# microsoft/VidTok

Hardware: AMD Instinct MI355X
Metric: encode+decode frames/sec, vidtok_kl_causal_488_4chn 17x256x256 (higher is better)
Workload: dtype bf16; 1 GPU; vidtok_kl_causal_488_4chn forward (encode+KL+decode), bf16, B=4 clips/GPU, 17x256x256; global_batch=4, launch=hipGraph replay (engine graph cache)

## Files before the change

### vidtok_amd/build.py

```python
import hashlib
import os
import re
import shutil
import subprocess
import sys

HERE = os.path.dirname(os.path.abspath(__file__))
CSRC = os.path.join(HERE, "csrc")
LIB = os.path.join(HERE, "libvidtok_amd.so")
SOURCES = ["conv_igemm_bf16.hip", "conv_igemm_f16.hip", "conv_igemm_f32.hip", "conv_igemm_x3.hip", "conv_igemm_act.hip", "conv_igemm.hip", "conv_in8.hip", "conv_ws2.hip", "conv_narrow.hip", "tblock_ws128.hip", "attention.hip", "pointwise.hip", "groupnorm.hip", "regularizers.hip", "metrics.hip", "lpips.hip", "lpips_grad.hip", "video_io.hip", "segments.hip", "grad.hip", "grad_decoder.hip", "patchgan.hip", "packing.hip", "error.cpp", "options.cpp", "model.cpp"]
HEADERS = ["common.h", "conv_common.h", "conv_rows.h", "conv_select.h", "conv_igemm_kernel.h", "launch.h", "options.h", "row8.h", os.path.join("..", "..", "include", "vidtok_amd.h")]
FLAGS = ["--offload-arch=gfx950", "-O3", "-std=c++17", "-fPIC", "-Wall", "-Wno-unused-function"]
EXTRA_FLAGS = {"conv_ws2.hip": ["-fno-slp-vectorize"], "tblock_ws128.hip": ["-fno-slp-vectorize"]}


NO_SPILL = {"tblock_ws128.hip": "tblock_pair_kernel", "conv_ws2.hip": "conv3x3_ws2_kernel", "conv_in8.hip": "conv_in8_kernel",
            "conv_igemm_bf16.hip": re.compile(r"conv_igemm_glds_kernel.*Lb[01]ELi2ELb0ELi\dELi0EEEvNS_8ConvArgsE$"),
            "conv_igemm_f16.hip": re.compile(r"conv_igemm_glds_kernel.*Lb[01]ELi2ELb0ELi\dELi0EEEvNS_8ConvArgsE$")}
PROF_LAST = ("tblock_pair_kernel", "conv3x3_ws2_kernel")
LLVM_BIN = "/opt/rocm/lib/llvm/bin"


def kernel_resources(obj):
    import re
    import tempfile
    with tempfile.TemporaryDirectory() as d:
        fat, dev = os.path.join(d, "fat.bin"), os.path.join(d, "dev.o")
        subprocess.check_call([f"{LLVM_BIN}/llvm-objcopy", "--dump-section", f".hip_fatbin={fat}", obj])
        subprocess.check_call([f"{LLVM_BIN}/clang-offload-bundler", "--unbundle", "--type=o", f"--input={fat}",
                               "--targets=hipv4-amdgcn-amd-amdhsa--gfx950", f"--output={dev}"])
        notes = subprocess.check_output([f"{LLVM_BIN}/llvm-readelf", "--notes", dev], text=True)
    out = []
    for blk in notes.split("- .agpr_count:")[1:]:
        g = lambda k: re.search(r"\." + k + r":\s+(\S+)", blk).group(1)
        out.append((g("name"), int(g("vgpr_count")), int(blk.split()[0]), int(g("vgpr_spill_count")), int(g("private_segment_fixed_size"))))
    return out


def check_no_spill(objdir):
    if not all(os.path.exists(os.path.join(LLVM_BIN, t)) for t in ("llvm-objcopy", "clang-offload-bundler", "llvm-readelf")):
        print("[vidtok_amd.build] spill check skipped: LLVM binutils not found under", LLVM_BIN, flush=True)
        return
    bad = []
    for src, kern in NO_SPILL.items():
        obj = os.path.join(objdir, os.path.splitext(src)[0] + ".o")
        for name, _v, _a, spill, scratch in kernel_resources(obj):
            measured = any(k in name for k in PROF_LAST) and name.endswith(("Lb1EEEvNS_10TBlockArgsE", "Lb1EEEvNS_8ConvArgsE"))
            hit = kern in name if isinstance(kern, str) else kern.search(name) is not None
            if hit and not measured and (spill or scratch):
                bad.append(f"{name}: {spill} spilled registers, {scratch} B scratch")
    if bad:
        raise RuntimeError("register spills in hand-scheduled kernels (wrong results, not only slow):\n  " + "\n  ".join(bad))


def _hipcc():
    for c in (os.environ.get("HIPCC"), shutil.which("hipcc"), "/opt/rocm/bin/hipcc"):
        if c and os.path.exists(c):
            return c
    raise RuntimeError("hipcc not found (set HIPCC)")


def _src_digest(src):
    h = hashlib.sha256()
    for f in [src] + HEADERS:
        with open(os.path.join(CSRC, f), "rb") as fh:
            h.update(fh.read())
    h.update(" ".join(FLAGS + EXTRA_FLAGS.get(src, [])).encode())
    return h.hexdigest()


def _digest():
    h = hashlib.sha256()
    for src in SOURCES:
        h.update(_src_digest(src).encode())
    return h.hexdigest()


def build(force: bool = False, verbose: bool = True) -> str:
    stamp = LIB + ".stamp"
    dig = _digest()
    if not force and os.path.exists(LIB) and os.path.exists(stamp) and open(stamp).read() == dig:
        return LIB
    hipcc = _hipcc()
    objdir = os.path.join(HERE, "build")
    os.makedirs(objdir, exist_ok=True)
    objs = []
    procs = []
    for src in SOURCES:
        obj = os.path.join(objdir, os.path.splitext(src)[0] + ".o")
        objs.append(obj)
        ostamp, odig = obj + ".stamp", _src_digest(src)
        if not force and os.path.exists(obj) and os.path.exists(ostamp) and open(ostamp).read() == odig:
            continue
        if os.path.exists(ostamp):
            os.remove(ostamp)
        cmd = [hipcc, *FLAGS, *EXTRA_FLAGS.get(src, []), "-x", "hip", "-c", os.path.join(CSRC, src), "-o", obj]
        if verbose:
            print("[vidtok_amd.build]", " ".join(cmd), flush=True)
        procs.append((src, subprocess.Popen(cmd), ostamp, odig))
    failed = []
    for src, p, ostamp, odig in procs:
        if p.wait() != 0:
            failed.append(src)
        else:
            with open(ostamp, "w") as f:
                f.write(odig)
    if failed:
        raise RuntimeError(f"hipcc failed on {', '.join(failed)}")
    check_no_spill(objdir)
    cmd = [hipcc, "--offload-arch=gfx950", "-shared", "-fPIC", *objs, "-o", LIB]
    if verbose:
        print("[vidtok_amd.build]", " ".join(cmd), flush=True)
    subprocess.check_call(cmd)
    with open(stamp, "w") as f:
        f.write(dig)
    return LIB


if __name__ == "__main__":
    build(force="--force" in sys.argv)
    print(LIB)
```

### vidtok_amd/csrc/attention.hip

```cpp
#include <atomic>

#include "conv_common.h"

namespace {

constexpr int FA_D = 512;
constexpr int FA_BQ = 64;
constexpr int FA_BK = 32;
constexpr int FA_KTILE = FA_BK * FA_D * 2;
constexpr int FA_VTILE = FA_D * FA_BK * 2;
constexpr int FA_STAGE = FA_KTILE + FA_VTILE;
constexpr int FA_LDS = 2 * FA_STAGE;

struct FlashArgs {
  const uint16_t* q;
  const uint16_t* k;
  const uint16_t* vt;
  const float* bias_v;
  uint16_t* o;
  int S, ldv;
  float scale_log2e;
};

template <typename H>
__global__ __launch_bounds__(256, 1) void flash_attn_kernel(const FlashArgs p) {
#if defined(__HIP_DEVICE_COMPILE__)
  extern __shared__ __attribute__((aligned(16))) char smem[];
  typedef __attribute__((address_space(3))) void* lds_ptr_t;
  const int lane = threadIdx.x & 63;
  const int wave = __builtin_amdgcn_readfirstlane(threadIdx.x >> 6);
  const int z = blockIdx.y, q0 = blockIdx.x * FA_BQ + wave * 16;
  const int S = p.S;
  const int n = lane & 15, g = lane >> 4;
  const uint16_t* qz = p.q + (long long)z * S * FA_D;
  const uint16_t* kz = p.k + (long long)z * S * FA_D;
  const uint16_t* vz = p.vt + (long long)z * FA_D * p.ldv;

  u32x4 qf[16];
#pragma unroll
  for (int ks = 0; ks < 16; ++ks) qf[ks] = *reinterpret_cast<const u32x4*>(qz + (long long)(q0 + n) * FA_D + ks * 32 + g * 8);

  const __amdgpu_buffer_rsrc_t rk = __builtin_amdgcn_make_buffer_rsrc(const_cast<uint16_t*>(kz), 0, (unsigned)S * FA_D * 2u, 0x00020000);
  const __amdgpu_buffer_rsrc_t rv = __builtin_amdgcn_make_buffer_rsrc(const_cast<uint16_t*>(vz), 0, (unsigned)FA_D * (unsigned)p.ldv * 2u, 0x00020000);
  auto issue_tile = [&](int t, int stg) {
    char* kd = smem + stg * FA_STAGE;
    char* vd = kd + FA_KTILE;
#pragma unroll
    for (int i = 0; i < 8; ++i) {
      const int r = wave * 8 + i;
      const unsigned off = (unsigned)(t * FA_BK + r) * (FA_D * 2u) + (unsigned)((lane ^ (r & 15)) * 16);
      __builtin_amdgcn_raw_ptr_buffer_load_lds(rk, (lds_ptr_t)(kd + r * 1024), 16, off, 0, 0, 0);
    }
#pragma unroll
    for (int j = 0; j < 8; ++j) {
      const int d = 16 * (wave * 8 + j) + (lane >> 2);
      const int c = (lane & 3) ^ ((d >> 2) & 3);
      const unsigned off = (unsigned)d * (unsigned)p.ldv * 2u + (unsigned)(t * FA_BK * 2 + c * 16);
      __builtin_amdgcn_raw_ptr_buffer_load_lds(rv, (lds_ptr_t)(vd + 16 * (wave * 8 + j) * 64), 16, off, 0, 0, 0);
    }
  };

  f32x4 acc[32];
#pragma unroll
  for (int mt = 0; mt < 32; ++mt) acc[mt] = f32x4{0.f, 0.f, 0.f, 0.f};
  float m_run = -3.0e38f, l_run = 0.f;

  const int ntile = S / FA_BK;
  issue_tile(0, 0);
  for (int t = 0; t < ntile; ++t) {
    const int stg = t & 1;
    wait_vmcnt<0>();
    __syncthreads();
    if (t + 1 < ntile) issue_tile(t + 1, stg ^ 1);
    const char* kt = smem + stg * FA_STAGE;
    const char* vt = kt + FA_KTILE;
    f32x4 s0 = f32x4{0.f, 0.f, 0.f, 0.f}, s1 = s0;
#pragma unroll
    for (int ks = 0; ks < 16; ++ks) {
      const int slot = ((4 * ks + g) ^ n) * 16;
      const u32x4 a0 = *reinterpret_cast<const u32x4*>(kt + n * 1024 + slot);
      const u32x4 a1 = *reinterpret_cast<const u32x4*>(kt + (16 + n) * 1024 + slot);
      s0 = h16<H>::mfma16(a0, qf[ks], s0);
      s1 = h16<H>::mfma16(a1, qf[ks], s1);
    }
    float v[8];
#pragma unroll
    for (int i = 0; i < 4; ++i) {
      v[i] = s0[i] * p.scale_log2e;
      v[4 + i] = s1[i] * p.scale_log2e;
    }
    float mx = v[0];
#pragma unroll
    for (int i = 1; i < 8; ++i) mx = fmaxf(mx, v[i]);
    mx = fmaxf(mx, __shfl_xor(mx, 16, 64));
    mx = fmaxf(mx, __shfl_xor(mx, 32, 64));
    const float m_new = fmaxf(m_run, mx);
    const float alpha = __builtin_amdgcn_exp2f(m_run - m_new);
    float ps = 0.f, pv[8];
#pragma unroll
    for (int i = 0; i < 8; ++i) {
      pv[i] = __builtin_amdgcn_exp2f(v[i] - m_new);
      ps += pv[i];
    }
    ps += __shfl_xor(ps, 16, 64);
    ps += __shfl_xor(ps, 32, 64);
    l_run = l_run * alpha + ps;
    m_run = m_new;
    u32x4 pf;
    pf[0] = h16<H>::pack(pv[0], pv[1]);
    pf[1] = h16<H>::pack(pv[2], pv[3]);
    pf[2] = h16<H>::pack(pv[4], pv[5]);
    pf[3] = h16<H>::pack(pv[6], pv[7]);
    if (__builtin_amdgcn_ballot_w64(alpha != 1.0f) != 0ull) {
#pragma unroll
      for (int mt = 0; mt < 32; ++mt)
#pragma unroll
        for (int i = 0; i < 4; ++i) acc[mt][i] *= alpha;
    }
#pragma unroll
    for (int mt = 0; mt < 32; ++mt) {
      const int d = 16 * mt + n;
      const int sw = (d >> 2) & 3;
      const char* row = vt + d * 64 + 8 * (g & 1);
      const u32x2 lo = *reinterpret_cast<const u32x2*>(row + (((g >> 1) ^ sw) * 16));
      const u32x2 hi = *reinterpret_cast<const u32x2*>(row + (((2 + (g >> 1)) ^ sw) * 16));
      const u32x4 a = u32x4{lo[0], lo[1], hi[0], hi[1]};
      acc[mt] = h16<H>::mfma16(a, pf, acc[mt]);
    }
  }
  const float inv = 1.0f / l_run;
  H* orow = reinterpret_cast<H*>(p.o) + ((long long)z * S + q0 + n) * FA_D;
#pragma unroll
  for (int mt = 0; mt < 32; ++mt) {
    const int d0 = 16 * mt + 4 * g;
    f32x4 b = f32x4{0.f, 0.f, 0.f, 0.f};
    if (p.bias_v) b = *reinterpret_cast<const f32x4*>(p.bias_v + d0);
    float o[4];
#pragma unroll
    for (int i = 0; i < 4; ++i) o[i] = acc[mt][i] * inv + b[i];
    store_quad<H>(orow + d0, o);
  }
#endif
}

}

extern "C" int vt_flash_attention_supported(int32_t dtype, int32_t S, int32_t C, int32_t ldv) {
  return vt_opt(OPT_ATTN_FLASH) != 0 && vt_is_h16(dtype) && C == FA_D && S > 0 && S % FA_BQ == 0 && ldv >= S && ldv % 8 == 0 &&
         (long long)S * FA_D * 2 < 0xFFFF0000ll && (long long)FA_D * ldv * 2 < 0xFFFF0000ll;
}

extern "C" int vt_flash_attention(const void* q, const void* k, const void* vt, const float* bias_v, void* o, int32_t dtype, int32_t Z, int32_t S,
                                  int32_t C, int32_t ldv, float scale, vt_stream stream_) {
  hipStream_t stream = reinterpret_cast<hipStream_t>(stream_);
  VT_CHECK_ARG(q && k && vt && o && Z > 0, "vt_flash_attention: null tensor or empty batch");
  VT_CHECK_ARG(vt_opt(OPT_ATTN_FLASH) != 0, "vt_flash_attention: switched off (option attn_flash = 0)");
  VT_CHECK_ARG(vt_flash_attention_supported(dtype, S, C, ldv), "vt_flash_attention: bf16 / fp16, C = 512, S %% 64 == 0, ldv >= S and %% 8 == 0 only (got dtype %d S %d C %d ldv %d)",
               dtype, S, C, ldv);
  const uintptr_t al = reinterpret_cast<uintptr_t>(q) | reinterpret_cast<uintptr_t>(k) | reinterpret_cast<uintptr_t>(vt) | reinterpret_cast<uintptr_t>(o) |
                       reinterpret_cast<uintptr_t>(bias_v);
  VT_CHECK_ARG((al & 15) == 0, "vt_flash_attention: tensors must be 16-byte aligned");
  FlashArgs a;
  a.q = (const uint16_t*)q; a.k = (const uint16_t*)k; a.vt = (const uint16_t*)vt; a.bias_v = bias_v; a.o = (uint16_t*)o;
  a.S = S; a.ldv = ldv;
  a.scale_log2e = scale * 1.4426950408889634f;
  const void* kern = dtype == VT_F16 ? reinterpret_cast<const void*>(&flash_attn_kernel<f16_t>) : reinterpret_cast<const void*>(&flash_attn_kernel<bf16_t>);
  const int ki = dtype == VT_F16 ? 1 : 0;
  static std::atomic<bool> attr_done[2][kMaxDevices];
  if (const int rc = vt_dynamic_lds(kern, FA_LDS, attr_done[ki])) return rc;
  for (int z0 = 0; z0 < Z; z0 += 65535) {
    const int zn = Z - z0 < 65535 ? Z - z0 : 65535;
    FlashArgs s = a;
    s.q = a.q + (long long)z0 * S * FA_D; s.k = a.k + (long long)z0 * S * FA_D; s.o = a.o + (long long)z0 * S * FA_D;
    s.vt = a.vt + (long long)z0 * FA_D * ldv;
    void* kargs[] = {&s};
    VT_CHECK_HIP(hipLaunchKernel(kern, dim3((unsigned)(S / FA_BQ), (unsigned)zn), dim3(256), kargs, FA_LDS, stream));
  }
  return VT_OK;
}
```

### vidtok_amd/csrc/conv_common.h

```cpp
#pragma once
#include "common.h"
#include "options.h"

namespace {

constexpr int kRowBytes = 128;

struct FastDiv {
  unsigned mul, shift, d;
};
inline FastDiv make_fastdiv(unsigned d) {
  FastDiv f;
  f.d = d;
  if (d <= 1) { f.mul = 0; f.shift = 0; return f; }
  unsigned l = 0;
  while ((1ull << l) < d) ++l;
  f.mul = (unsigned)((((1ull << 32) * ((1ull << l) - d)) / d) + 1);
  f.shift = l - 1;
  return f;
}
__device__ __forceinline__ unsigned fast_div(unsigned n, const FastDiv& f) {
  if (f.d <= 1) return n;
  const unsigned t = __umulhi(n, f.mul);
  return (t + ((n - t) >> 1)) >> f.shift;
}

struct ConvArgs;
__device__ __forceinline__ long long out_row(const ConvArgs& p, int m);

struct ConvArgs {
  const char* x;
  const char* w;
  const float* bias;
  char* y;
  const char* res;
  const char* cache;
  const float* mix_factor;
  const float* ln_gamma;
  const float* ln_beta;
  char* ln_out;
  int B, Ti, Hi, Wi, Cin;
  int To, Ho, Wo, Cout;
  int ldw, ldy;
  int KT, KH, KW;
  int st, sh, sw;
  int pt, ph, pw;
  int tmode, ncache;
  int ups_t, ups_s;
  int res_mode, res_tshift, Tr, ldr;
  int out_layout, t_trim;
  int M, K, ntaps, nsteps;
  int m_tiles, n_tiles;
  int ln_mode, ln_keep_y, ldn;
  float ln_eps;
  FastDiv fd_wo, fd_ho, fd_to;
  FastDiv fd_hw;
  int yt_mul;
  long long yt_step, yt_base;
  int ys_mul, ys_oh, ys_ow;
  int lds_epi;
  int hw_tiles;
  unsigned x_bytes, w_bytes;
  unsigned c_bytes;
  long long xs_z, ws_z, ys_z, rs_z;
  int in8_rt, in8_ct, in8_ctl2, in8_segs;
  int tskip;
  int ksplit;
  unsigned plane_bytes;
  int nt_store;
  unsigned long long* prof;
  int prof_mode;
  const char* pair_v;
  int ldv;
};

struct split3_t {
  float v;
};
template <typename MT>
struct is_split3 {
  [[maybe_unused]] static constexpr bool value = false;
};
template <>
struct is_split3<split3_t> {
  [[maybe_unused]] static constexpr bool value = true;
};
template <typename MT>
struct storage_of {
  typedef MT type;
};
template <>
struct storage_of<split3_t> {
  typedef float type;
};

__device__ __forceinline__ void split3_x(const u32x4& r0, const u32x4& r1, u32x4& hi, u32x4& lo) {
#pragma unroll
  for (int e = 0; e < 4; ++e) {
    const float f0 = __uint_as_float(e < 2 ? r0[2 * e] : r1[2 * e - 4]);
    const float f1 = __uint_as_float(e < 2 ? r0[2 * e + 1] : r1[2 * e - 3]);
    const uint32_t h = pack_bf16x2(f0, f1);
    hi[e] = h;
    float d0, d1;
    asm("v_sub_f32_e32 %0, %1, %2" : "=v"(d0) : "v"(f0), "v"(h << 16));
    asm("v_sub_f32_e32 %0, %1, %2" : "=v"(d1) : "v"(f1), "v"(h & 0xffff0000u));
    lo[e] = pack_bf16x2(d0, d1);
  }
}
__device__ __forceinline__ void mma_bf16(const u32x4& wfrag, const u32x4& xfrag, f32x16& acc) {
  acc = __builtin_amdgcn_mfma_f32_32x32x16_bf16(__builtin_bit_cast(bf16x8, wfrag), __builtin_bit_cast(bf16x8, xfrag), acc, 0, 0, 0);
}

template <typename MT>
__device__ __forceinline__ void mma_step(const u32x4& wfrag, const u32x4& xfrag, f32x16& acc);

template <>
__device__ __forceinline__ void mma_step<bf16_t>(const u32x4& wfrag, const u32x4& xfrag, f32x16& acc) {
  acc = __builtin_amdgcn_mfma_f32_32x32x16_bf16(__builtin_bit_cast(bf16x8, wfrag),
                                                __builtin_bit_cast(bf16x8, xfrag), acc, 0, 0, 0);
}
template <>
__device__ __forceinline__ void mma_step<f16_t>(const u32x4& wfrag, const u32x4& xfrag, f32x16& acc) {
  acc = h16<f16_t>::mfma32(wfrag, xfrag, acc);
}
template <>
__device__ __forceinline__ void mma_step<float>(const u32x4& wfrag, const u32x4& xfrag, f32x16& acc) {
#pragma unroll
  for (int e = 0; e < 4; ++e)
    acc = __builtin_amdgcn_mfma_f32_32x32x2f32(__uint_as_float(wfrag[e]), __uint_as_float(xfrag[e]),
                                               acc, 0, 0, 0);
}

__device__ __forceinline__ int xcd_remap(int bid, int nblk) {
  const int xcd = bid & 7, loc = bid >> 3;
  const int q = nblk >> 3, r = nblk & 7;
  const int start = (xcd < r) ? xcd * (q + 1) : r * (q + 1) + (xcd - r) * q;
  return start + loc;
}

template <typename TOut>
struct Quad;
template <>
struct Quad<float> {
  f32x4 v;
  __device__ __forceinline__ float get(int e) const { return v[e]; }
};
template <typename H>
struct Quad16 {
  u32x2 v;
  __device__ __forceinline__ float get(int e) const {
    const uint32_t w = v[e >> 1];
    return (e & 1) ? h16<H>::hi(w) : h16<H>::lo(w);
  }
};
template <>
struct Quad<bf16_t> : Quad16<bf16_t> {};
template <>
struct Quad<f16_t> : Quad16<f16_t> {};
template <typename TOut>
__device__ __forceinline__ void store_quad(TOut* p, const float (&v)[4]);
template <>
__device__ __forceinline__ void store_quad<float>(float* p, const float (&v)[4]) {
  f32x4 t;
  t[0] = v[0]; t[1] = v[1]; t[2] = v[2]; t[3] = v[3];
  *reinterpret_cast<f32x4*>(p) = t;
}
template <>
__device__ __forceinline__ void store_quad<bf16_t>(bf16_t* p, const float (&v)[4]) {
  u32x2 t;
  t[0] = h16<bf16_t>::pack(v[0], v[1]);
  t[1] = h16<bf16_t>::pack(v[2], v[3]);
  *reinterpret_cast<u32x2*>(p) = t;
}
template <>
__device__ __forceinline__ void store_quad<f16_t>(f16_t* p, const float (&v)[4]) {
  u32x2 t;
  t[0] = h16<f16_t>::pack(v[0], v[1]);
  t[1] = h16<f16_t>::pack(v[2], v[3]);
  *reinterpret_cast<u32x2*>(p) = t;
}

template <typename TOut>
struct Oct;
__device__ __forceinline__ void store16_nt(void* p, const u32x4& v) {
  asm volatile("global_store_dwordx4 %0, %1, off nt\n\ts_nop 1" ::"v"(p), "v"(v) : "memory");
}

template <>
struct Oct<float> {
  f32x4 lo, hi;
  __device__ __forceinline__ void load(const float* p) {
    lo = *reinterpret_cast<const f32x4*>(p);
    hi = *reinterpret_cast<const f32x4*>(p + 4);
  }
  __device__ __forceinline__ float get(int e) const { return e < 4 ? lo[e] : hi[e - 4]; }
  static __device__ __forceinline__ void store(float* p, const float (&v)[8], bool nt = false) {
    f32x4 a, b;
#pragma unroll
    for (int e = 0; e < 4; ++e) { a[e] = v[e]; b[e] = v[4 + e]; }
    if (nt) {
      store16_nt(p, __builtin_bit_cast(u32x4, a));
      store16_nt(p + 4, __builtin_bit_cast(u32x4, b));
    } else {
      *reinterpret_cast<f32x4*>(p) = a;
      *reinterpret_cast<f32x4*>(p + 4) = b;
    }
  }
};
template <typename H>
struct Oct16 {
  u32x4 w;
  __device__ __forceinline__ void load(const H* p) { w = *reinterpret_cast<const u32x4*>(p); }
  __device__ __forceinline__ float get(int e) const {
    const uint32_t t = w[e >> 1];
    return (e & 1) ? h16<H>::hi(t) : h16<H>::lo(t);
  }
  static __device__ __forceinline__ void store(H* p, const float (&v)[8], bool nt = false) {
    u32x4 t;
// ... 33 lines not shown
```

### vidtok_amd/csrc/conv_in8.hip

```cpp
#include <atomic>
#include <type_traits>

#include "conv_select.h"
#include "conv_rows.h"

namespace {

template <int I, int N, typename F>
__device__ __forceinline__ void static_for(F&& f) {
  if constexpr (I < N) {
    f(std::integral_constant<int, I>{});
    static_for<I + 1, N>(f);
  }
}

constexpr int kIn8TBytes = 64 * 128 * 4;

template <typename TOut>
__device__ __forceinline__ void conv_epilogue_in8(const ConvArgs& p, f32x16 (&acc)[4], int m_blk, int wave, int lane, int tid, char* smem) {
  static_assert(sizeof(TOut) == 2, "conv_in8_kernel: 16-bit storage");
  TOut* __restrict__ yg = reinterpret_cast<TOut*>(p.y);
  TOut* __restrict__ ng = reinterpret_cast<TOut*>(p.ln_out);
  float* T = reinterpret_cast<float*>(smem);
  const int oct_j = tid & 15;
  const int row0 = tid >> 4;
  float lg[8], lb[8];
  if (p.ln_mode) rows_affine(p, oct_j, p.ln_mode == 2, lg, lb);
  static_for<0, 2>([&](auto pc) __attribute__((always_inline)) {
    constexpr int pass = decltype(pc)::value;
    __syncthreads();
#pragma unroll
    for (int g = 0; g < 4; ++g) {
      const int c = 32 * wave + 8 * g + 4 * (lane >> 5);
      const f32x4 bq = rows_bias(p.bias, c);
#pragma unroll
      for (int bl = 0; bl < 2; ++bl) rows_scatter<128>(T, bl * 32 + (lane & 31), c, acc[2 * pass + bl], g, bq);
    }
    __syncthreads();
#pragma unroll
    for (int it = 0; it < 4; ++it) {
      const int row = row0 + 16 * it;
      float v[8];
      rows_read<128>(T, row, oct_j, v);
      const long long orow = out_row(p, m_blk + 64 * pass + row);
      rows_finish<16, TOut, 0>(p, VT_RES_NONE, v, Oct<TOut>{}, 0.0f, lg, lb, yg + orow * p.ldy + 8 * oct_j, ng + orow * p.ldn + 8 * oct_j);
    }
  });
}

template <typename H, bool REPL>
__global__ __launch_bounds__(256, 2) void conv_in8_kernel(const ConvArgs p) {
#if defined(__HIP_DEVICE_COMPILE__)
  extern __shared__ __attribute__((aligned(16))) char smem[];
  typedef __attribute__((address_space(3))) void* lds_ptr_t;
  const int tid = threadIdx.x;
  const int lane = tid & 63;
  const int wave = __builtin_amdgcn_readfirstlane(tid >> 6);
  const int half = lane >> 5, l32 = lane & 31;
  const int tile = xcd_remap(blockIdx.x, gridDim.x);
  const int m_blk = tile * 128;
  const unsigned fi = fast_div((unsigned)m_blk, p.fd_hw);
  const int rem = m_blk - (int)fi * (p.Ho * p.Wo);
  const int h0 = (int)fast_div((unsigned)rem, p.fd_wo);
  const int w0 = rem - h0 * p.Wo;
  const int bb = (int)fast_div(fi, p.fd_to);
  const int t = (int)fi - bb * p.To;
  const int CT = p.in8_ct, SEGS = p.in8_segs;
  const int PR = p.in8_rt + 2, RS = SEGS * 64;
  char* patch = smem + kIn8TBytes;
  const int zslot = 3 * PR * RS * 16;

  const __amdgpu_buffer_rsrc_t rx = __builtin_amdgcn_make_buffer_rsrc(const_cast<char*>(p.x), 0, p.x_bytes, 0x00020000);
  const int nq = 3 * PR * SEGS;
  for (int q = wave; q < nq; q += 4) {
    const int prow = q / SEGS, seg = q - prow * SEGS;
    const int f = prow / PR, r = prow - f * PR;
    const int tt = t + f - 2, hh = h0 + r - 1;
    const int c = seg * 64 + lane;
    const int ww = w0 + c - 1;
    const bool ok = (c < CT + 2) & ((unsigned)ww < (unsigned)p.Wi) & ((unsigned)hh < (unsigned)p.Hi) & (REPL | (tt >= 0));
    const unsigned off = ok ? (unsigned)(((bb * p.Ti + max(tt, 0)) * p.Hi + hh) * p.Wi + ww) * 16u : 0xFFFF0000u;
    __builtin_amdgcn_raw_ptr_buffer_load_lds(rx, (lds_ptr_t)(patch + (prow * RS + seg * 64) * 16), 16, off, 0, 0, 0);
  }
  if (tid == 0) *reinterpret_cast<u32x4*>(patch + zslot) = u32x4{0u, 0u, 0u, 0u};

  u32x4 wf[14];
  {
    const H* row = reinterpret_cast<const H*>(p.w) + (long long)(32 * wave + l32) * p.ldw + 8 * half;
#pragma unroll
    for (int j = 0; j < 14; ++j) {
      if (j < 13 || half == 0) wf[j] = *reinterpret_cast<const u32x4*>(row + 16 * j);
      else wf[j] = u32x4{0u, 0u, 0u, 0u};
    }
  }
  int fb[4];
#pragma unroll
  for (int b = 0; b < 4; ++b) {
    const int pix = b * 32 + l32;
    const int pr = pix >> p.in8_ctl2, pc = pix & (CT - 1);
    fb[b] = (pr * RS + pc) * 16;
  }
  wait_vmcnt<0>();
  __syncthreads();

  f32x16 acc[4];
  constexpr int PF = 2;
  u32x4 xf[PF + 1][4];
  auto issue = [&](auto jc) __attribute__((always_inline)) {
    constexpr int j = decltype(jc)::value;
    constexpr int tpa = 2 * j, tpb = 2 * j + 1;
    const int da = (((tpa / 9) * PR + (tpa % 9) / 3) * RS + tpa % 3) * 16;
    const int db = tpb < 27 ? (((tpb / 9) * PR + (tpb % 9) / 3) * RS + tpb % 3) * 16 : 0;
#pragma unroll
    for (int b = 0; b < 4; ++b) {
      int a = fb[b] + (half ? db : da);
      if (tpb >= 27) a = half ? zslot : a;
      xf[j % (PF + 1)][b] = *reinterpret_cast<const u32x4*>(patch + a);
    }
  };
  static_for<0, PF>([&](auto jc) __attribute__((always_inline)) { issue(jc); });
  static_for<0, 14>([&](auto jc) __attribute__((always_inline)) {
    constexpr int j = decltype(jc)::value;
    if constexpr (j + PF < 14) issue(std::integral_constant<int, j + PF>{});
#pragma unroll
    for (int b = 0; b < 4; ++b) {
      if constexpr (std::is_same<H, bf16_t>::value) {
        if constexpr (j == 0) asm volatile("v_mfma_f32_32x32x16_bf16 %0, %1, %2, 0" : "=&a"(acc[b]) : "a"(wf[j]), "v"(xf[j % (PF + 1)][b]));
        else asm volatile("v_mfma_f32_32x32x16_bf16 %0, %1, %2, %0" : "+a"(acc[b]) : "a"(wf[j]), "v"(xf[j % (PF + 1)][b]));
      } else {
        if constexpr (j == 0) asm volatile("v_mfma_f32_32x32x16_f16 %0, %1, %2, 0" : "=&a"(acc[b]) : "a"(wf[j]), "v"(xf[j % (PF + 1)][b]));
        else asm volatile("v_mfma_f32_32x32x16_f16 %0, %1, %2, %0" : "+a"(acc[b]) : "a"(wf[j]), "v"(xf[j % (PF + 1)][b]));
      }
    }
    __builtin_amdgcn_sched_barrier(0);
  });
  asm volatile("s_nop 15\n\ts_nop 3" ::: "memory");
  conv_epilogue_in8<H>(p, acc, m_blk, wave, lane, tid, smem);
#endif
}


}

extern "C" __attribute__((visibility("hidden"))) int vt_conv_in8_launch(const void* args, int dtype, void* stream_) {
  hipStream_t stream = reinterpret_cast<hipStream_t>(stream_);
  ConvArgs a = *reinterpret_cast<const ConvArgs*>(args);
  a.x_bytes = (unsigned)gather_extents(a, 2).x;
  a.in8_ct = a.Wo >= 128 ? 128 : a.Wo;
  a.in8_rt = 128 / a.in8_ct;
  a.in8_segs = (a.in8_ct + 2 + 63) / 64;
  a.in8_ctl2 = 0;
  while ((1 << a.in8_ctl2) < a.in8_ct) ++a.in8_ctl2;
  const int tiles = a.M / 128;
  const int lds = kIn8TBytes + 3 * (a.in8_rt + 2) * a.in8_segs * 64 * 16 + 16;
  static const void* const kerns[4] = {reinterpret_cast<const void*>(&conv_in8_kernel<bf16_t, false>), reinterpret_cast<const void*>(&conv_in8_kernel<bf16_t, true>),
                                       reinterpret_cast<const void*>(&conv_in8_kernel<f16_t, false>), reinterpret_cast<const void*>(&conv_in8_kernel<f16_t, true>)};
  const int ki = (dtype == VT_F16 ? 2 : 0) + (a.tmode == VT_TPAD_REPLICATE ? 1 : 0);
  static std::atomic<bool> attr_done[4][kMaxDevices];
  if (const int rc = vt_dynamic_lds(kerns[ki], 160 * 1024, attr_done[ki])) return rc;
  void* kargs[] = {&a};
  VT_CHECK_HIP(hipLaunchKernel(kerns[ki], dim3((unsigned)tiles), dim3(256), kargs, lds, stream));
  return VT_OK;
}
```

### vidtok_amd/csrc/regularizers.hip

```cpp
#include <math.h>

#include "launch.h"

namespace {

constexpr int kBlock = 256;
constexpr int kMaxD = 8;
constexpr int kMaxL = 16;

__global__ __launch_bounds__(1024) void kl_sample_kernel(const float* __restrict__ h, const float* __restrict__ noise,
                                                         float* __restrict__ z, float* __restrict__ kl_out, int B,
                                                         int zc, long long S) {
  __shared__ float red[16];
  const long long per_b = (long long)zc * S;
  const long long n = (long long)B * per_b;
  float acc = 0.f;
  for (long long i = threadIdx.x; i < n; i += 1024) {
    const long long b = i / per_b;
    const long long r = i - b * per_b;
    const float mean = h[b * 2 * per_b + r];
    float logvar = h[b * 2 * per_b + per_b + r];
    logvar = fminf(fmaxf(logvar, -30.0f), 20.0f);
    const float stdv = expf(0.5f * logvar);
    const float var = expf(logvar);
    z[i] = noise ? mean + stdv * noise[i] : mean;
    acc += mean * mean + var - 1.0f - logvar;
  }
  acc = wave_sum(acc, 64);
  if ((threadIdx.x & 63) == 0) red[threadIdx.x >> 6] = acc;
  __syncthreads();
  if (threadIdx.x < 64) {
    float v = threadIdx.x < 16 ? red[threadIdx.x] : 0.f;
    v = wave_sum(v, 64);
    if (threadIdx.x == 0) kl_out[0] = 0.5f * v / (float)B;
  }
}

struct FsqConsts {
  int D;
  int levels[kMaxD];
  int basis[kMaxD];
  float half_l[kMaxD];
  float offset[kMaxD];
  float shift[kMaxD];
  float half_w[kMaxD];
};

__device__ __forceinline__ float tanh_cr(float x) { return (float)tanh((double)x); }

__device__ __forceinline__ float fsq_round(float zv, float shift, float half_l, float offset) {
  const float t = tanh_cr(__fadd_rn(zv, shift));
  const float bounded = __fsub_rn(__fmul_rn(t, half_l), offset);
  return rintf(bounded);
}

__global__ __launch_bounds__(kBlock) void fsq_quantize_kernel(const float* __restrict__ h, float* __restrict__ z,
                                                              int* __restrict__ indices, FsqConsts k, int B,
                                                              long long S, int ncb) {
  const long long n = (long long)B * S;
  for (long long i = (long long)blockIdx.x * kBlock + threadIdx.x; i < n; i += (long long)gridDim.x * kBlock) {
    const long long b = i / S, s = i - b * S;
    int idx = 0;
    for (int d = 0; d < k.D; ++d) {
      const float q = fsq_round(h[(b * k.D + d) * S + s], k.shift[d], k.half_l[d], k.offset[d]);
      z[(b * k.D + d) * S + s] = q / k.half_w[d];
      idx += ((int)q + k.levels[d] / 2) * k.basis[d];
    }
    indices[ncb == 1 ? i : ((b / ncb) * S + s) * ncb + (b % ncb)] = idx;
  }
}

__global__ __launch_bounds__(kBlock) void fsq_indices_to_codes_kernel(const int* __restrict__ indices,
                                                                      float* __restrict__ z, FsqConsts k, int B,
                                                                      long long S, int ncb) {
  const long long n = (long long)B * S;
  for (long long i = (long long)blockIdx.x * kBlock + threadIdx.x; i < n; i += (long long)gridDim.x * kBlock) {
    const long long b = i / S, s = i - b * S;
    const int idx = indices[ncb == 1 ? i : ((b / ncb) * S + s) * ncb + (b % ncb)];
    for (int d = 0; d < k.D; ++d) {
      const int lv = (idx / k.basis[d]) % k.levels[d];
      z[(b * k.D + d) * S + s] = ((float)lv - k.half_w[d]) / k.half_w[d];
    }
  }
}

__global__ __launch_bounds__(kBlock) void fsq_aux_tables_kernel(const float* __restrict__ h, FsqConsts k, int B,
                                                                long long S, float inv_temp,
                                                                float* __restrict__ tables, float* __restrict__ accum) {
  const long long n = (long long)B * S;
  float commit = 0.f;
  for (long long i = (long long)blockIdx.x * kBlock + threadIdx.x; i < n; i += (long long)gridDim.x * kBlock) {
    const long long b = i / S, s = i - b * S;
    for (int d = 0; d < k.D; ++d) {
      const float zv = h[(b * k.D + d) * S + s];
      const float q = fsq_round(zv, k.shift[d], k.half_l[d], k.offset[d]);
      const float code = q / k.half_w[d];
      commit += (zv - code) * (zv - code);
      float* t = tables + (i * k.D + d) * kMaxL;
      const int L = k.levels[d];
      float mx = -INFINITY;
      for (int l = 0; l < L; ++l) {
        const float c = ((float)l - k.half_w[d]) / k.half_w[d];
        const float logit = 2.0f * inv_temp * zv * c;
        t[l] = logit;
        mx = fmaxf(mx, logit);
      }
      float sum = 0.f;
      for (int l = 0; l < L; ++l) {
        const float e = expf(t[l] - mx);
        t[l] = e;
        sum += e;
      }
      const float inv = 1.0f / sum;
      for (int l = 0; l < L; ++l) t[l] *= inv;
    }
  }
  commit = wave_sum(commit, 64);
  if ((threadIdx.x & 63) == 0) atomicAdd(accum + 2, commit);
}

constexpr int kTokTiles = 64;
constexpr int kHiChunk = 16;
constexpr int kTokSub = 32;

struct FsqSplit {
  int dl;
  int JL, JH;
};
inline FsqSplit fsq_split(const FsqConsts& k) {
  FsqSplit s;
  s.dl = 0;
  s.JL = 1;
  while (s.dl < k.D - 1 && s.JL * k.levels[s.dl] <= 512) s.JL *= k.levels[s.dl++];
  if (s.dl == 0) s.JL = k.levels[s.dl++];
  s.JH = 1;
  for (int d = s.dl; d < k.D; ++d) s.JH *= k.levels[d];
  return s;
}

__global__ __launch_bounds__(kBlock) void fsq_aux_pairs_kernel(const float* __restrict__ tables, FsqConsts k, FsqSplit sp,
                                                               long long ntok, long long tile_tokens, int J,
                                                               float* __restrict__ part, float* __restrict__ accum) {
  __shared__ float tab[kTokSub][kMaxD][kMaxL];
  __shared__ float hi[kTokSub][kHiChunk];
  const int tile = blockIdx.x;
  const int hc0 = blockIdx.y * kHiChunk;
  const long long t_begin = (long long)tile * tile_tokens;
  const long long t_end = min(t_begin + tile_tokens, ntok);
  constexpr int kLowPerThread = 2;
  int lo_off[kLowPerThread][kMaxD];
  bool lo_ok[kLowPerThread];
#pragma unroll
  for (int u = 0; u < kLowPerThread; ++u) {
    int jl = threadIdx.x + u * kBlock;
    lo_ok[u] = jl < sp.JL;
#pragma unroll
    for (int d = 0; d < kMaxD; ++d) {
      const int L = d < sp.dl ? k.levels[d] : 1;
      lo_off[u][d] = lo_ok[u] ? jl % L : 0;
      jl /= L;
    }
  }
  float acc[kLowPerThread][kHiChunk];
#pragma unroll
  for (int u = 0; u < kLowPerThread; ++u)
#pragma unroll
    for (int h = 0; h < kHiChunk; ++h) acc[u][h] = 0.f;
  float ent = 0.f;
  for (long long t0 = t_begin; t0 < t_end; t0 += kTokSub) {
    const int nt = (int)min((long long)kTokSub, t_end - t0);
    __syncthreads();
    for (int i = threadIdx.x; i < nt * k.D * kMaxL; i += kBlock) {
      const int tt = i / (k.D * kMaxL), r = i - tt * (k.D * kMaxL);
      tab[tt][r / kMaxL][r % kMaxL] = tables[(t0 + tt) * k.D * kMaxL + r];
    }
    __syncthreads();
    for (int i = threadIdx.x; i < nt * kHiChunk; i += kBlock) {
      const int tt = i / kHiChunk, h = i - tt * kHiChunk;
      int jh = hc0 + h;
// ... 236 lines not shown
```

Before: 993.6 frames/s.

## Persistent double-buffered in8 conv, 512-thread flash attention, unrolled KL sampling

The in8 first-layer conv becomes a persistent kernel capped at twice the CU count. It double-buffers halo patches in LDS so the next tile's gather overlaps the current tile's MFMA work, and it keeps bias and layer-norm affine values in LDS and registers. Flash attention now launches 512 threads, with two wave groups each owning half of the head dimension, which halves the per-wave accumulators and the K/V tile loads per wave. The single-block KL sampling kernel is unrolled eight-way so loads are batched before compute, and the per-element division is replaced with incremental indexing. The changes add complexity and register-pressure risk, so a spill check is added for the attention kernel.

```diff
diff --git a/vidtok_amd/build.py b/vidtok_amd/build.py
--- a/vidtok_amd/build.py
+++ b/vidtok_amd/build.py
@@ -15,6 +15,7 @@
 
 
 NO_SPILL = {"tblock_ws128.hip": "tblock_pair_kernel", "conv_ws2.hip": "conv3x3_ws2_kernel", "conv_in8.hip": "conv_in8_kernel",
+            "attention.hip": "flash_attn_kernel",
             "conv_igemm_bf16.hip": re.compile(r"conv_igemm_glds_kernel.*Lb[01]ELi2ELb0ELi\dELi0EEEvNS_8ConvArgsE$"),
             "conv_igemm_f16.hip": re.compile(r"conv_igemm_glds_kernel.*Lb[01]ELi2ELb0ELi\dELi0EEEvNS_8ConvArgsE$")}
 PROF_LAST = ("tblock_pair_kernel", "conv3x3_ws2_kernel")
diff --git a/vidtok_amd/csrc/attention.hip b/vidtok_amd/csrc/attention.hip
--- a/vidtok_amd/csrc/attention.hip
+++ b/vidtok_amd/csrc/attention.hip
@@ -23,13 +23,14 @@
 };
 
 template <typename H>
-__global__ __launch_bounds__(256, 1) void flash_attn_kernel(const FlashArgs p) {
+__global__ __launch_bounds__(512, 1) void flash_attn_kernel(const FlashArgs p) {
 #if defined(__HIP_DEVICE_COMPILE__)
   extern __shared__ __attribute__((aligned(16))) char smem[];
   typedef __attribute__((address_space(3))) void* lds_ptr_t;
   const int lane = threadIdx.x & 63;
   const int wave = __builtin_amdgcn_readfirstlane(threadIdx.x >> 6);
-  const int z = blockIdx.y, q0 = blockIdx.x * FA_BQ + wave * 16;
+  const int dh = wave >> 2;
+  const int z = blockIdx.y, q0 = blockIdx.x * FA_BQ + (wave & 3) * 16;
   const int S = p.S;
   const int n = lane & 15, g = lane >> 4;
   const uint16_t* qz = p.q + (long long)z * S * FA_D;
@@ -46,23 +47,23 @@
     char* kd = smem + stg * FA_STAGE;
     char* vd = kd + FA_KTILE;
 #pragma unroll
-    for (int i = 0; i < 8; ++i) {
-      const int r = wave * 8 + i;
+    for (int i = 0; i < 4; ++i) {
+      const int r = wave * 4 + i;
       const unsigned off = (unsigned)(t * FA_BK + r) * (FA_D * 2u) + (unsigned)((lane ^ (r & 15)) * 16);
       __builtin_amdgcn_raw_ptr_buffer_load_lds(rk, (lds_ptr_t)(kd + r * 1024), 16, off, 0, 0, 0);
     }
 #pragma unroll
-    for (int j = 0; j < 8; ++j) {
-      const int d = 16 * (wave * 8 + j) + (lane >> 2);
+    for (int j = 0; j < 4; ++j) {
+      const int d = 16 * (wave * 4 + j) + (lane >> 2);
       const int c = (lane & 3) ^ ((d >> 2) & 3);
       const unsigned off = (unsigned)d * (unsigned)p.ldv * 2u + (unsigned)(t * FA_BK * 2 + c * 16);
-      __builtin_amdgcn_raw_ptr_buffer_load_lds(rv, (lds_ptr_t)(vd + 16 * (wave * 8 + j) * 64), 16, off, 0, 0, 0);
+      __builtin_amdgcn_raw_ptr_buffer_load_lds(rv, (lds_ptr_t)(vd + 16 * (wave * 4 + j) * 64), 16, off, 0, 0, 0);
     }
   };
 
-  f32x4 acc[32];
+  f32x4 acc[16];
 #pragma unroll
-  for (int mt = 0; mt < 32; ++mt) acc[mt] = f32x4{0.f, 0.f, 0.f, 0.f};
+  for (int mt = 0; mt < 16; ++mt) acc[mt] = f32x4{0.f, 0.f, 0.f, 0.f};
   float m_run = -3.0e38f, l_run = 0.f;
 
   const int ntile = S / FA_BK;
@@ -113,13 +114,13 @@
     pf[3] = h16<H>::pack(pv[6], pv[7]);
     if (__builtin_amdgcn_ballot_w64(alpha != 1.0f) != 0ull) {
 #pragma unroll
-      for (int mt = 0; mt < 32; ++mt)
+      for (int mt = 0; mt < 16; ++mt)
 #pragma unroll
         for (int i = 0; i < 4; ++i) acc[mt][i] *= alpha;
     }
 #pragma unroll
-    for (int mt = 0; mt < 32; ++mt) {
-      const int d = 16 * mt + n;
+    for (int mt = 0; mt < 16; ++mt) {
+      const int d = 16 * (16 * dh + mt) + n;
       const int sw = (d >> 2) & 3;
       const char* row = vt + d * 64 + 8 * (g & 1);
       const u32x2 lo = *reinterpret_cast<const u32x2*>(row + (((g >> 1) ^ sw) * 16));
@@ -131,8 +132,8 @@
   const float inv = 1.0f / l_run;
   H* orow = reinterpret_cast<H*>(p.o) + ((long long)z * S + q0 + n) * FA_D;
 #pragma unroll
-  for (int mt = 0; mt < 32; ++mt) {
-    const int d0 = 16 * mt + 4 * g;
+  for (int mt = 0; mt < 16; ++mt) {
+    const int d0 = 16 * (16 * dh + mt) + 4 * g;
     f32x4 b = f32x4{0.f, 0.f, 0.f, 0.f};
     if (p.bias_v) b = *reinterpret_cast<const f32x4*>(p.bias_v + d0);
     float o[4];
@@ -174,7 +175,7 @@
     s.q = a.q + (long long)z0 * S * FA_D; s.k = a.k + (long long)z0 * S * FA_D; s.o = a.o + (long long)z0 * S * FA_D;
     s.vt = a.vt + (long long)z0 * FA_D * ldv;
     void* kargs[] = {&s};
-    VT_CHECK_HIP(hipLaunchKernel(kern, dim3((unsigned)(S / FA_BQ), (unsigned)zn), dim3(256), kargs, FA_LDS, stream));
+    VT_CHECK_HIP(hipLaunchKernel(kern, dim3((unsigned)(S / FA_BQ), (unsigned)zn), dim3(512), kargs, FA_LDS, stream));
   }
   return VT_OK;
 }
diff --git a/vidtok_amd/csrc/conv_common.h b/vidtok_amd/csrc/conv_common.h
--- a/vidtok_amd/csrc/conv_common.h
+++ b/vidtok_amd/csrc/conv_common.h
@@ -63,7 +63,7 @@
   unsigned x_bytes, w_bytes;
   unsigned c_bytes;
   long long xs_z, ws_z, ys_z, rs_z;
-  int in8_rt, in8_ct, in8_ctl2, in8_segs;
+  int in8_rt, in8_ct, in8_ctl2, in8_pieces;
   int tskip;
   int ksplit;
   unsigned plane_bytes;
diff --git a/vidtok_amd/csrc/conv_in8.hip b/vidtok_amd/csrc/conv_in8.hip
--- a/vidtok_amd/csrc/conv_in8.hip
+++ b/vidtok_amd/csrc/conv_in8.hip
@@ -15,28 +15,33 @@
 }
 
 constexpr int kIn8TBytes = 64 * 128 * 4;
+constexpr int kIn8PSlots = 5;
+
+__device__ __forceinline__ void in8_lds_barrier() {
+  asm volatile("s_waitcnt lgkmcnt(0)" ::: "memory");
+  __builtin_amdgcn_s_barrier();
+}
 
 template <typename TOut>
-__device__ __forceinline__ void conv_epilogue_in8(const ConvArgs& p, f32x16 (&acc)[4], int m_blk, int wave, int lane, int tid, char* smem) {
+__device__ __forceinline__ void conv_epilogue_in8(const ConvArgs& p, f32x16 (&acc)[4], int m_blk, int wave, int lane, int tid, char* smem,
+                                                  const float* bias_lds, const float (&lg)[8], const float (&lb)[8]) {
   static_assert(sizeof(TOut) == 2, "conv_in8_kernel: 16-bit storage");
   TOut* __restrict__ yg = reinterpret_cast<TOut*>(p.y);
   TOut* __restrict__ ng = reinterpret_cast<TOut*>(p.ln_out);
   float* T = reinterpret_cast<float*>(smem);
   const int oct_j = tid & 15;
   const int row0 = tid >> 4;
-  float lg[8], lb[8];
-  if (p.ln_mode) rows_affine(p, oct_j, p.ln_mode == 2, lg, lb);
   static_for<0, 2>([&](auto pc) __attribute__((always_inline)) {
     constexpr int pass = decltype(pc)::value;
-    __syncthreads();
+    in8_lds_barrier();
 #pragma unroll
     for (int g = 0; g < 4; ++g) {
       const int c = 32 * wave + 8 * g + 4 * (lane >> 5);
-      const f32x4 bq = rows_bias(p.bias, c);
+      const f32x4 bq = *reinterpret_cast<const f32x4*>(bias_lds + c);
 #pragma unroll
       for (int bl = 0; bl < 2; ++bl) rows_scatter<128>(T, bl * 32 + (lane & 31), c, acc[2 * pass + bl], g, bq);
     }
-    __syncthreads();
+    in8_lds_barrier();
 #pragma unroll
     for (int it = 0; it < 4; ++it) {
       const int row = row0 + 16 * it;
@@ -57,32 +62,44 @@
   const int lane = tid & 63;
   const int wave = __builtin_amdgcn_readfirstlane(tid >> 6);
   const int half = lane >> 5, l32 = lane & 31;
-  const int tile = xcd_remap(blockIdx.x, gridDim.x);
-  const int m_blk = tile * 128;
-  const unsigned fi = fast_div((unsigned)m_blk, p.fd_hw);
-  const int rem = m_blk - (int)fi * (p.Ho * p.Wo);
-  const int h0 = (int)fast_div((unsigned)rem, p.fd_wo);
-  const int w0 = rem - h0 * p.Wo;
-  const int bb = (int)fast_div(fi, p.fd_to);
-  const int t = (int)fi - bb * p.To;
-  const int CT = p.in8_ct, SEGS = p.in8_segs;
-  const int PR = p.in8_rt + 2, RS = SEGS * 64;
-  char* patch = smem + kIn8TBytes;
-  const int zslot = 3 * PR * RS * 16;
+  const int CT = p.in8_ct;
+  const int PR = p.in8_rt + 2, RS = CT + 2;
+  const int slot_bytes = p.in8_pieces * 1024;
+  char* const patch0 = smem + kIn8TBytes;
+  char* const zero16 = patch0 + 2 * slot_bytes;
+  const int ntiles = p.M >> 7, grid = (int)gridDim.x;
 
   const __amdgpu_buffer_rsrc_t rx = __builtin_amdgcn_make_buffer_rsrc(const_cast<char*>(p.x), 0, p.x_bytes, 0x00020000);
-  const int nq = 3 * PR * SEGS;
-  for (int q = wave; q < nq; q += 4) {
-    const int prow = q / SEGS, seg = q - prow * SEGS;
+  int geo[kIn8PSlots];
+#pragma unroll
+  for (int k = 0; k < kIn8PSlots; ++k) {
+    const int fp = (wave + 4 * k) * 64 + lane;
+    const int prow = fp / RS, c = fp - prow * RS;
     const int f = prow / PR, r = prow - f * PR;
-    const int tt = t + f - 2, hh = h0 + r - 1;
-    const int c = seg * 64 + lane;
-    const int ww = w0 + c - 1;
-    const bool ok = (c < CT + 2) & ((unsigned)ww < (unsigned)p.Wi) & ((unsigned)hh < (unsigned)p.Hi) & (REPL | (tt >= 0));
-    const unsigned off = ok ? (unsigned)(((bb * p.Ti + max(tt, 0)) * p.Hi + hh) * p.Wi + ww) * 16u : 0xFFFF0000u;
-    __builtin_amdgcn_raw_ptr_buffer_load_lds(rx, (lds_ptr_t)(patch + (prow * RS + seg * 64) * 16), 16, off, 0, 0, 0);
+    geo[k] = f < 3 ? (c | (r << 8) | (f << 16)) : (1 << 20);
   }
-  if (tid == 0) *reinterpret_cast<u32x4*>(patch + zslot) = u32x4{0u, 0u, 0u, 0u};
+  auto request_patch = [&](int v, int slot) __attribute__((always_inline)) {
+    const int m0 = xcd_remap(v, ntiles) * 128;
+    const unsigned fi = fast_div((unsigned)m0, p.fd_hw);
+    const int rem = m0 - (int)fi * (p.Ho * p.Wo);
+    const int h0 = (int)fast_div((unsigned)rem, p.fd_wo);
+    const int w0 = rem - h0 * p.Wo;
+    const int bb = (int)fast_div(fi, p.fd_to);
+    const int t = (int)fi - bb * p.To;
+    char* dst = patch0 + slot * slot_bytes;
+#pragma unroll
+    for (int k = 0; k < kIn8PSlots; ++k) {
+      if (wave + 4 * k < p.in8_pieces) {
+        const int c = geo[k] & 255, r = (geo[k] >> 8) & 255, f = geo[k] >> 16;
+        const int tt = t + f - 2, hh = h0 + r - 1, ww = w0 + c - 1;
+        const bool ok = (f < 3) & ((unsigned)ww < (unsigned)p.Wi) & ((unsigned)hh < (unsigned)p.Hi) & (REPL | (tt >= 0));
+        const unsigned off = ok ? (unsigned)(((bb * p.Ti + max(tt, 0)) * p.Hi + hh) * p.Wi + ww) * 16u : 0xFFFF0000u;
+        __builtin_amdgcn_raw_ptr_buffer_load_lds(rx, (lds_ptr_t)(dst + (wave + 4 * k) * 1024), 16, off, 0, 0, 0);
+      }
+    }
+  };
+  request_patch((int)blockIdx.x, 0);
+  if (tid == 0) *reinterpret_cast<u32x4*>(zero16) = u32x4{0u, 0u, 0u, 0u};
 
   u32x4 wf[14];
   {
@@ -93,6 +110,12 @@
       else wf[j] = u32x4{0u, 0u, 0u, 0u};
     }
   }
+  float* const bias_lds = reinterpret_cast<float*>(zero16 + 16);
+  if (tid < 128) bias_lds[tid] = p.bias ? p.bias[tid] : 0.0f;
+  float lg[8], lb[8];
+#pragma unroll
+  for (int e = 0; e < 8; ++e) lg[e] = lb[e] = 0.0f;
+  if (p.ln_mode) rows_affine(p, tid & 15, p.ln_mode == 2, lg, lb);
   int fb[4];
 #pragma unroll
   for (int b = 0; b < 4; ++b) {
@@ -100,42 +123,52 @@
     const int pr = pix >> p.in8_ctl2, pc = pix & (CT - 1);
     fb[b] = (pr * RS + pc) * 16;
   }
-  wait_vmcnt<0>();
-  __syncthreads();
+  const bool two_stores = p.ln_mode != 0 && p.ln_keep_y != 0;
 
-  f32x16 acc[4];
-  constexpr int PF = 2;
-  u32x4 xf[PF + 1][4];
-  auto issue = [&](auto jc) __attribute__((always_inline)) {
-    constexpr int j = decltype(jc)::value;
-    constexpr int tpa = 2 * j, tpb = 2 * j + 1;
-    const int da = (((tpa / 9) * PR + (tpa % 9) / 3) * RS + tpa % 3) * 16;
-    const int db = tpb < 27 ? (((tpb / 9) * PR + (tpb % 9) / 3) * RS + tpb % 3) * 16 : 0;
+  int slot = 0;
+  for (int v = (int)blockIdx.x; v < ntiles; v += grid, slot ^= 1) {
+    if (v == (int)blockIdx.x) wait_vmcnt<0>();
+    else if (two_stores) wait_vmcnt<16>();
+    else wait_vmcnt<8>();
+    in8_lds_barrier();
+    if (v + grid < ntiles) request_patch(v + grid, slot ^ 1);
+    const char* patch = patch0 + slot * slot_bytes;
+    const int m_blk = xcd_remap(v, ntiles) * 128;
+
+    f32x16 acc[4];
+    constexpr int PF = 2;
+    u32x4 xf[PF + 1][4];
+    auto issue = [&](auto jc) __attribute__((always_inline)) {
+      constexpr int j = decltype(jc)::value;
+      constexpr int tpa = 2 * j, tpb = 2 * j + 1;
+      const int da = (((tpa / 9) * PR + (tpa % 9) / 3) * RS + tpa % 3) * 16;
+      const int db = tpb < 27 ? (((tpb / 9) * PR + (tpb % 9) / 3) * RS + tpb % 3) * 16 : 0;
 #pragma unroll
-    for (int b = 0; b < 4; ++b) {
-      int a = fb[b] + (half ? db : da);
-      if (tpb >= 27) a = half ? zslot : a;
-      xf[j % (PF + 1)][b] = *reinterpret_cast<const u32x4*>(patch + a);
-    }
-  };
-  static_for<0, PF>([&](auto jc) __attribute__((always_inline)) { issue(jc); });
-  static_for<0, 14>([&](auto jc) __attribute__((always_inline)) {
-    constexpr int j = decltype(jc)::value;
-    if constexpr (j + PF < 14) issue(std::integral_constant<int, j + PF>{});
+      for (int b = 0; b < 4; ++b) {
+        const char* a = patch + fb[b] + (half ? db : da);
+        if (tpb >= 27) a = half ? zero16 : a;
+        xf[j % (PF + 1)][b] = *reinterpret_cast<const u32x4*>(a);
+      }
+    };
+    static_for<0, PF>([&](auto jc) __attribute__((always_inline)) { issue(jc); });
+    static_for<0, 14>([&](auto jc) __attribute__((always_inline)) {
+      constexpr int j = decltype(jc)::value;
+      if constexpr (j + PF < 14) issue(std::integral_constant<int, j + PF>{});
 #pragma unroll
-    for (int b = 0; b < 4; ++b) {
-      if constexpr (std::is_same<H, bf16_t>::value) {
-        if constexpr (j == 0) asm volatile("v_mfma_f32_32x32x16_bf16 %0, %1, %2, 0" : "=&a"(acc[b]) : "a"(wf[j]), "v"(xf[j % (PF + 1)][b]));
-        else asm volatile("v_mfma_f32_32x32x16_bf16 %0, %1, %2, %0" : "+a"(acc[b]) : "a"(wf[j]), "v"(xf[j % (PF + 1)][b]));
-      } else {
-        if constexpr (j == 0) asm volatile("v_mfma_f32_32x32x16_f16 %0, %1, %2, 0" : "=&a"(acc[b]) : "a"(wf[j]), "v"(xf[j % (PF + 1)][b]));
-        else asm volatile("v_mfma_f32_32x32x16_f16 %0, %1, %2, %0" : "+a"(acc[b]) : "a"(wf[j]), "v"(xf[j % (PF + 1)][b]));
+      for (int b = 0; b < 4; ++b) {
+        if constexpr (std::is_same<H, bf16_t>::value) {
+          if constexpr (j == 0) asm volatile("v_mfma_f32_32x32x16_bf16 %0, %1, %2, 0" : "=&a"(acc[b]) : "a"(wf[j]), "v"(xf[j % (PF + 1)][b]));
+          else asm volatile("v_mfma_f32_32x32x16_bf16 %0, %1, %2, %0" : "+a"(acc[b]) : "a"(wf[j]), "v"(xf[j % (PF + 1)][b]));
+        } else {
+          if constexpr (j == 0) asm volatile("v_mfma_f32_32x32x16_f16 %0, %1, %2, 0" : "=&a"(acc[b]) : "a"(wf[j]), "v"(xf[j % (PF + 1)][b]));
+          else asm volatile("v_mfma_f32_32x32x16_f16 %0, %1, %2, %0" : "+a"(acc[b]) : "a"(wf[j]), "v"(xf[j % (PF + 1)][b]));
+        }
       }
-    }
-    __builtin_amdgcn_sched_barrier(0);
-  });
-  asm volatile("s_nop 15\n\ts_nop 3" ::: "memory");
-  conv_epilogue_in8<H>(p, acc, m_blk, wave, lane, tid, smem);
+      __builtin_amdgcn_sched_barrier(0);
+    });
+    asm volatile("s_nop 15\n\ts_nop 3" ::: "memory");
+    conv_epilogue_in8<H>(p, acc, m_blk, wave, lane, tid, smem, bias_lds, lg, lb);
+  }
 #endif
 }
 
@@ -148,17 +181,19 @@
   a.x_bytes = (unsigned)gather_extents(a, 2).x;
   a.in8_ct = a.Wo >= 128 ? 128 : a.Wo;
   a.in8_rt = 128 / a.in8_ct;
-  a.in8_segs = (a.in8_ct + 2 + 63) / 64;
+  a.in8_pieces = (3 * (a.in8_rt + 2) * (a.in8_ct + 2) + 63) / 64;
+  VT_CHECK_ARG(a.in8_pieces <= 4 * kIn8PSlots, "conv_in8: a halo patch of %d pieces (at most %d)", a.in8_pieces, 4 * kIn8PSlots);
   a.in8_ctl2 = 0;
   while ((1 << a.in8_ctl2) < a.in8_ct) ++a.in8_ctl2;
   const int tiles = a.M / 128;
-  const int lds = kIn8TBytes + 3 * (a.in8_rt + 2) * a.in8_segs * 64 * 16 + 16;
+  const int grid = tiles < 2 * device_cus() ? tiles : 2 * device_cus();
+  const int lds = kIn8TBytes + 2 * a.in8_pieces * 1024 + 16 + 128 * 4;
   static const void* const kerns[4] = {reinterpret_cast<const void*>(&conv_in8_kernel<bf16_t, false>), reinterpret_cast<const void*>(&conv_in8_kernel<bf16_t, true>),
                                        reinterpret_cast<const void*>(&conv_in8_kernel<f16_t, false>), reinterpret_cast<const void*>(&conv_in8_kernel<f16_t, true>)};
   const int ki = (dtype == VT_F16 ? 2 : 0) + (a.tmode == VT_TPAD_REPLICATE ? 1 : 0);
   static std::atomic<bool> attr_done[4][kMaxDevices];
   if (const int rc = vt_dynamic_lds(kerns[ki], 160 * 1024, attr_done[ki])) return rc;
   void* kargs[] = {&a};
-  VT_CHECK_HIP(hipLaunchKernel(kerns[ki], dim3((unsigned)tiles), dim3(256), kargs, lds, stream));
+  VT_CHECK_HIP(hipLaunchKernel(kerns[ki], dim3((unsigned)grid), dim3(256), kargs, lds, stream));
   return VT_OK;
 }
diff --git a/vidtok_amd/csrc/regularizers.hip b/vidtok_amd/csrc/regularizers.hip
--- a/vidtok_amd/csrc/regularizers.hip
+++ b/vidtok_amd/csrc/regularizers.hip
@@ -7,6 +7,16 @@
 constexpr int kBlock = 256;
 constexpr int kMaxD = 8;
 constexpr int kMaxL = 16;
+
+constexpr int kKlUnroll = 8;
+
+__device__ __forceinline__ float kl_element(float mean, float logvar, bool has_noise, float nz, float* __restrict__ zp) {
+  logvar = fminf(fmaxf(logvar, -30.0f), 20.0f);
+  const float stdv = expf(0.5f * logvar);
+  const float var = expf(logvar);
+  *zp = has_noise ? mean + stdv * nz : mean;
+  return mean * mean + var - 1.0f - logvar;
+}
 
 __global__ __launch_bounds__(1024) void kl_sample_kernel(const float* __restrict__ h, const float* __restrict__ noise,
                                                          float* __restrict__ z, float* __restrict__ kl_out, int B,
@@ -15,16 +25,34 @@
   const long long per_b = (long long)zc * S;
   const long long n = (long long)B * per_b;
   float acc = 0.f;
-  for (long long i = threadIdx.x; i < n; i += 1024) {
-    const long long b = i / per_b;
-    const long long r = i - b * per_b;
-    const float mean = h[b * 2 * per_b + r];
-    float logvar = h[b * 2 * per_b + per_b + r];
-    logvar = fminf(fmaxf(logvar, -30.0f), 20.0f);
-    const float stdv = expf(0.5f * logvar);
-    const float var = expf(logvar);
-    z[i] = noise ? mean + stdv * noise[i] : mean;
-    acc += mean * mean + var - 1.0f - logvar;
+  long long i = threadIdx.x;
+  long long b = i / per_b;
+  long long r = i - b * per_b;
+  auto advance = [&]() {
+    i += 1024;
+    r += 1024;
+    if (r >= per_b) {
+      const long long q = r / per_b;
+      b += q;
+      r -= q * per_b;
+    }
+  };
+  while (i + (long long)(kKlUnroll - 1) * 1024 < n) {
+    float mean[kKlUnroll], logvar[kKlUnroll], nz[kKlUnroll];
+    const long long i0 = i;
+#pragma unroll
+    for (int j = 0; j < kKlUnroll; ++j) {
+      mean[j] = h[b * 2 * per_b + r];
+      logvar[j] = h[b * 2 * per_b + per_b + r];
+      nz[j] = noise ? noise[i] : 0.f;
+      advance();
+    }
+#pragma unroll
+    for (int j = 0; j < kKlUnroll; ++j) acc += kl_element(mean[j], logvar[j], noise != nullptr, nz[j], z + i0 + (long long)j * 1024);
+  }
+  while (i < n) {
+    acc += kl_element(h[b * 2 * per_b + r], h[b * 2 * per_b + per_b + r], noise != nullptr, noise ? noise[i] : 0.f, z + i);
+    advance();
   }
   acc = wave_sum(acc, 64);
   if ((threadIdx.x & 63) == 0) red[threadIdx.x >> 6] = acc;
```

After: 1000 frames/s (median of 6 runs). About the same (+0.7%).
